# real-stanford/dgdm

Measured on AMD Instinct MI355X. Metric: guided samples/sec (full DDIM chain), higher is better.
Workload: dtype f32_split_f16x3; 1 GPU; 3d_guided BASELINE configs[2] (configs[3] at 8 GPUs): B=32 G=45 P=5 R=36000 sub_bs=512 N=512 T=15/S=5, fresh object per pair; contraction_flag=f32, fingers_per_pair=32, denoise_steps=5, rows_per_cond_fn=36000, cond_fn_per_chain_step=1, eps_net_form=f32_f16x3 batched, parallelism=pairs-sharded x1

## Files before the change

dgdm_amd/csrc/guidance_api.hip:

```cpp
#include "common.h"
#include "models.h"
#include <algorithm>
#include <cmath>
#include <cstring>
#include <unordered_map>
#include <atomic>
#include <thread>

using namespace dgdm;

namespace {

std::vector<float> linspace_f32(float start, float end, int steps) {
    std::vector<float> v(steps);
    if (steps == 1) { v[0] = start; return v; }
    const float step = (end - start) / (float)(steps - 1);
    const int half = steps / 2;
    for (int i = 0; i < steps; ++i) v[i] = i < half ? start + step * (float)i : end - step * (float)(steps - i - 1);
    return v;
}

struct ObjectTables {
    const float *xyz = nullptr;
    const int   *fps1 = nullptr;
// ... 40 lines not shown
    DevBuf pool_fps1t;
    DevBuf tmpY[NBUILD], tmpL2[NBUILD], vlist;
    DevBuf tmpShare[NBUILD];
    hipStream_t bstream[NBUILD] = {};
    hipEvent_t bev[NBUILD] = {}, bstart = nullptr, pooled = nullptr, ldone = nullptr;
    DevBuf V, genc, atab, chainbias, timepart, ttmp, ttmp64, partial, objdev, objidx, xobj, xobj16, starts, order, xchains, todo, groupoff;
    DevBuf loopx[2], loopeps, loopgrad, loopxrep, loopts;
    DevBuf loopeps1;
    DevBuf loopkeys;
    std::vector<uint64_t> loopkeys_host;
    DevBuf loopcond, loopx2, loopeps2;
    DevBuf scorelogits;
    DevBuf valobj;
    DevBuf sweep_ori, rollstate, rolllogits, rolltiles, rollpmax;
    const float *rowfield = nullptr;
    int rowfield_chains = 0;
    DevBuf pos_lin, goalspecs;
    DevBuf labelx, labelcounts, labelsums, labelfinal, labelfirst, labelleft, labelobj;
    int rolltiles_chains = 0;
    DevBuf xidx, xidxchains, xtabptrs;
    DevBuf l1ptrs, l1objs;
    bool l1tab = true;
    int fill_l1ptrs(const std::vector<const ObjectTables *> &of_chain, int *n_tabled, hipStream_t s);
    bool xtab_enabled = true;
    int xtab_policy = 0;
    int grads_since_set = 0;
    static constexpr int XTAB_AFTER = 5;
    int l2_gather_mode = 0;
    int xobj_mode = 0;
    int n_objects = 0;
    bool force_slow_xobj = false;
    void *pinned = nullptr; size_t pinned_bytes = 0; hipEvent_t pinned_ev = nullptr;
    int64_t todo_capacity = 0;
    int *ro_host = nullptr; size_t ro_ints = 0; hipEvent_t ro_ev = nullptr; bool ro_pending = false;
    int finish_objects();
    hipStream_t cstream = nullptr; hipEvent_t up_ready = nullptr, up_consumed = nullptr; bool consumed_recorded = false;
    int serial = 0;
    bool tables_off_stream() const { return !(serial & 3) && !prof_on(); }
    bool eps_beside() const { return !(serial & 5) && !prof_on(); }
    bool hoist_x_only() const { return !(serial & 1) && !prof_on(); }
    bool built_off_stream = false, join_pending = false, built_once = false;
    hipStream_t joined_stream = nullptr;
    hipEvent_t fork_ev = nullptr, side_ev = nullptr;
    int join_tables(hipStream_t s) {
        if (!built_off_stream || (!join_pending && s == joined_stream)) return DGDM_OK;
        DGDM_HIP_CHECK(hipStreamWaitEvent(s, ro_ev, 0));
        join_pending = false; joined_stream = s;
        return DGDM_OK;
    }
    int side_stream(hipStream_t *side) {
        if (!bstream[0]) DGDM_HIP_CHECK(hipStreamCreateWithFlags(&bstream[0], hipStreamNonBlocking));
        if (!fork_ev) DGDM_HIP_CHECK(hipEventCreateWithFlags(&fork_ev, hipEventDisableTiming));
        if (!side_ev) DGDM_HIP_CHECK(hipEventCreateWithFlags(&side_ev, hipEventDisableTiming));
        *side = bstream[0];
        return DGDM_OK;
    }
    ~DgdmGuidance() {
        for (int i = 0; i < NBUILD; ++i)
            if (bstream[i]) (void)hipStreamSynchronize(bstream[i]);
        if (fork_ev) (void)hipEventDestroy(fork_ev);
        if (side_ev) (void)hipEventDestroy(side_ev);
        if (pinned) (void)hipHostFree(pinned);
        if (pinned_ev) (void)hipEventDestroy(pinned_ev);
        if (ro_host) (void)hipHostFree(ro_host);
        if (ro_ev) (void)hipEventDestroy(ro_ev);
        if (cstream) (void)hipStreamDestroy(cstream);
        if (up_ready) (void)hipEventDestroy(up_ready);
        if (up_consumed) (void)hipEventDestroy(up_consumed);
        for (int i = 0; i < NBUILD; ++i) {
            if (bstream[i]) (void)hipStreamDestroy(bstream[i]);
            if (bev[i]) (void)hipEventDestroy(bev[i]);
        }
        if (bstart) (void)hipEventDestroy(bstart);
        if (ldone) (void)hipEventDestroy(ldone);
        if (pooled) (void)hipEventDestroy(pooled);
    }
    int build_pose_table(const std::vector<float> &ori, const std::vector<float> &pos, PoseGrid *dst, hipStream_t s);
    void set_grid(dgdm::TrunkParams *p, const PoseGrid &g, int n_chains) const;
    int check_objects(const int *oidx, int n_chains) const;
    bool tables_wanted() const { return xtab_enabled && !force_slow_xobj && xobj_mode == 0; }
    int common_pre(const float *x_dev, float t_scaled, const int *objidx_host, int n_chains, hipStream_t s);
    int upload_starts(const int64_t *starts_host, int n_chains, int64_t rows, hipStream_t s, bool need_order = true, int n_calls = 1,
                      int64_t call_stride = 0);
    int ensure_rows(int n_chains, int64_t rows_per_chain);
    int use_xtab(const int *objidx_host, int n_chains, int64_t rows, bool want16, int *l1, hipStream_t s);
    int build_object(int oi, int slot, hipStream_t s);
    int build_xtab(int oi, hipStream_t s);
    int run_xobj(const int *objidx_host, int n_chains, int64_t rows, bool want16, bool *used16, bool *via_tab, int *l1, hipStream_t s);
    struct Embedded {
        bool tab = false, used16 = false;
        int l1 = 0;
        int64_t rows_per_chain = 0;
        void point(dgdm::TrunkParams *p, const DgdmGuidance &g, int call, int64_t rows_per_call) const;
    };
    int embed_rows(const int *objidx_host, int n_chains, const int64_t *starts_host, int64_t rows_per_call, int n_calls, int64_t call_stride,
                   bool want16, Embedded *e, hipStream_t s);
    int embed(const int *objidx_host, int n_chains, const int64_t *starts_host, int n_calls, int64_t call_stride, Embedded *e, hipStream_t s);
    int trunk_front(int kind, const float *x_dev, int timestep, const int *objidx_host, const int64_t *starts_host, int n_chains, const Embedded *emb,
                    int call, dgdm::TrunkParams *p, hipStream_t s, bool pre_done = false);
};

int DgdmGuidance::build_pose_table(const std::vector<float> &ori, const std::vector<float> &pos, PoseGrid *dst, hipStream_t s) {
    const int n = (int)ori.size(), W1 = m->W1;
    dst->cells = n; dst->tiles_per_b = (n + 31) / 32; dst->rows = (int64_t)B * n;
    DevBuf d_ori, d_pos, d_emb;
    int rc;
    if ((rc = d_ori.upload(ori.data(), sizeof(float) * n))) return rc;
    if ((rc = d_pos.upload(pos.data(), sizeof(float) * 2 * n))) return rc;
    if ((rc = d_emb.alloc(sizeof(float) * 27 * n))) return rc;
    if ((rc = dst->tab.alloc(sizeof(float) * (size_t)W1 * n))) return rc;
    if ((rc = pose_embed(d_ori.as<float>(), d_pos.as<float>(), d_emb.as<float>(), n, s))) return rc;
    if ((rc = linear64(d_emb.as<float>(), nullptr, 27, m->blob64.at(m->off64.w1p_wt), nullptr, nullptr, 1, nullptr, dst->tab.as<float>(), W1, n, 27, W1, ACT_NONE, s))) return rc;
    if ((rc = dst->tiled.alloc(sizeof(float) * (size_t)W1 * dst->tiles_per_b * 32))) return rc;
    if ((rc = tile_table(dst->tab.as<float>(), n, W1, dst->tiled.as<float>(), s))) return rc;
    DGDM_HIP_CHECK(hipStreamSynchronize(s));
    return DGDM_OK;
// ... 232 lines not shown
            (rc = g->pool_pairs.alloc(no * N * N * sizeof(int))) || (rc = g->pool_rank.alloc(no * N * N * sizeof(short))) ||
            (rc = g->pool_F1.alloc(no * N * 128 * 8)) || (rc = g->pool_U.alloc(no * N * 128 * 8)) ||
            (rc = g->pool_fps1t.alloc(no * N * 64 * sizeof(uint4))))
            return rc;
        const bool l1 = g->l1tab && !g->bf16 && N >= 128;
        const size_t l1mo = (size_t)std::max(1, g->cfg.max_objects);
        if (l1) {
            std::vector<const void *> ptrs(3 * l1mo, nullptr);
            for (int i = 0; i < (int)g->tables.size(); ++i) {
                ObjectTables &t = *g->tables[i];
                if ((rc = t.M0.alloc((size_t)N * 256 * 4)) || (rc = t.L1Z.alloc((size_t)N * 512 * 4)) || (rc = t.L1K.alloc((size_t)N * sizeof(int)))) return rc;
                ptrs[i] = t.M0.p; ptrs[l1mo + i] = t.L1Z.p; ptrs[2 * l1mo + i] = t.L1K.p;
            }
            if ((rc = g->l1objs.alloc(sizeof(void *) * ptrs.size()))) return rc;
            DGDM_HIP_CHECK(hipMemcpyAsync(g->l1objs.p, ptrs.data(), sizeof(void *) * ptrs.size(), hipMemcpyHostToDevice, s));
        }
        for (int i = 0; i < n_objects; ++i) g->tables[i]->has_l1 = l1;
        if (!g->pooled) DGDM_HIP_CHECK(hipEventCreateWithFlags(&g->pooled, hipEventDisableTiming));
        DGDM_HIP_CHECK(hipMemcpyAsync(g->pool_xyz.p, objects_dev, no * N * 3 * 4, hipMemcpyDeviceToDevice, s));
        DGDM_HIP_CHECK(hipEventRecord(g->pooled, s));
        hipStream_t fs = s;
        if (off) {
            fs = g->bstream[ns - 1];
            for (int i = 1; i < ns; ++i) {
                DGDM_HIP_CHECK(hipStreamWaitEvent(g->bstream[i], g->pooled, 0));
                if (g->built_once) DGDM_HIP_CHECK(hipStreamWaitEvent(g->bstream[i], g->ro_ev, 0));
            }
        }
        if ((rc = pn_fps_tables(g->pool_xyz.as<float>(), N, N, g->pool_fps1.as<int>(), g->pool_fps2.as<int>(), g->pool_flags.as<int>(), fs, n_objects)))
            return rc;
        if (!g->bf16 && !g->l2_gather_mode && N <= 512 &&
            (rc = pn_fps_transpose(g->pool_fps1.as<int>(), N, g->pool_fps1t.as<uint4>(), fs, n_objects))) return rc;
        DGDM_HIP_CHECK(hipEventRecord(g->bstart, fs));
        for (int i = 0; i < n_objects; ++i) {
            ObjectTables &t = *g->tables[i];
            t.xyz = g->pool_xyz.as<float>() + (size_t)i * N * 3; t.fps1 = g->pool_fps1.as<int>() + (size_t)i * N * 512;
            t.fps2 = g->pool_fps2.as<int>() + (size_t)i * N * 128; t.flags = g->pool_flags.as<int>() + (size_t)i * N;
            t.crowded = g->pool_crowded.as<int>() + (size_t)i * N; t.clist = g->pool_clist.as<int>() + (size_t)i * (N + 1);
        }
        {
            hipStream_t ls = g->bstream[0];
            DGDM_HIP_CHECK(hipStreamWaitEvent(ls, g->pooled, 0));
            const PnWeights w = g->m->pn();
            if ((rc = pn_crowd(g->pool_xyz.as<float>(), N, w, g->pool_crowded.as<int>(), g->pool_clist.as<int>(), g->pool_clist.as<int>() + N,
                               g->pool_off.as<int>(), g->pool_pairs.as<int>(), g->pool_rank.as<short>(), ls, g->pool_ncr.as<int>(), n_objects)))
                return rc;
            if (g->bf16) {
                if ((rc = pn_sa1(g->pool_xyz.as<float>(), N, w, g->pool_F1.as<float>(), ls, n_objects))) return rc;
                if ((rc = linear(g->pool_F1.as<float>(), 128, w.sa2_wf_t, w.sa2_b0, nullptr, 1, g->pool_U.as<float>(), 128, n_objects * N, 128, 128,
                                 ACT_NONE, false, ls))) return rc;
            } else {
                const PnWeights64 w64 = g->m->pn64();
                if ((rc = pn_sa1_64(g->pool_xyz.as<float>(), N, w.r1sq, w64, g->pool_F1.as<double>(), ls, n_objects))) return rc;
                if ((rc = linear64(nullptr, g->pool_F1.as<double>(), 128, w64.sa2_wf_t, w64.sa2_b0, nullptr, 1, g->pool_U.as<double>(), nullptr, 128,
                                   n_objects * N, 128, 128, ACT_NONE, ls))) return rc;
            }
            DGDM_HIP_CHECK(hipEventRecord(g->ldone, ls));
        }
        for (int i = 0; i < nb; ++i) {
            DGDM_HIP_CHECK(hipStreamWaitEvent(g->bstream[i], g->bstart, 0));
            DGDM_HIP_CHECK(hipStreamWaitEvent(g->bstream[i], g->ldone, 0));
        }
        for (int i = 0; i < n_objects; ++i)
            if ((rc = g->build_object(i, i % nb, g->bstream[i % nb]))) return rc;
        hipStream_t es = off ? g->bstream[0] : s;
        for (int i = off ? 1 : 0; i < nb; ++i) {
            DGDM_HIP_CHECK(hipEventRecord(g->bev[i], g->bstream[i]));
            DGDM_HIP_CHECK(hipStreamWaitEvent(es, g->bev[i], 0));
        }
        if (l1) {
            void *const *po = g->l1objs.as<void *>();
            if ((rc = trunk_f16l_l1_tables(reinterpret_cast<const float *const *>(po), g->pool_ncr.as<int>(), reinterpret_cast<float *const *>(po + l1mo),
                                           reinterpret_cast<int *const *>(po + 2 * l1mo), N, n_objects, g->m->fwdh(), es))) return rc;
        }
        prof_end(s, DGDM_STAGE_TABLES, 0.0);
        const size_t need = no * N + no;
        if (need > g->ro_ints) {
            if (g->ro_host) DGDM_HIP_CHECK(hipHostFree(g->ro_host));
            g->ro_host = nullptr;
            DGDM_HIP_CHECK(hipHostMalloc(reinterpret_cast<void **>(&g->ro_host), need * sizeof(int), hipHostMallocDefault));
            g->ro_ints = need;
        }
        if (!g->ro_ev) DGDM_HIP_CHECK(hipEventCreateWithFlags(&g->ro_ev, hipEventDisableTiming));
        DGDM_HIP_CHECK(hipMemcpyAsync(g->ro_host, g->pool_flags.p, sizeof(int) * no * N, hipMemcpyDeviceToHost, es));
        DGDM_HIP_CHECK(hipMemcpyAsync(g->ro_host + no * N, g->pool_ncr.p, sizeof(int) * no, hipMemcpyDeviceToHost, es));
        DGDM_HIP_CHECK(hipEventRecord(g->ro_ev, es));
        g->ro_pending = true;
        g->built_once = true; g->built_off_stream = off; g->join_pending = off;
    }
    g->n_objects = n_objects;
    g->grads_since_set = 0;
    return DGDM_OK;
}

int DgdmGuidance::common_pre(const float *x_dev, float t_scaled, const int *objidx_host, int n_chains, hipStream_t s) {
    const int rows = n_chains * B, W1 = m->W1;
    int rc;
    if ((rc = m->gripper_forward64(x_dev, m->L, V.as<double>(), genc.as<double>(), rows, s))) return rc;
    if ((rc = m->time_part64(t_scaled, ttmp.as<float>(), ttmp64.as<double>(), timepart.as<double>(), s))) return rc;
    if (m->kind == 2) {
        DGDM_HIP_CHECK(hipMemcpyAsync(objidx.p, objidx_host, sizeof(int) * n_chains, hipMemcpyHostToDevice, s));
        if ((rc = gather_add64(objpart.as<double>(), objidx.as<int>(), timepart.as<double>(), chainbias.as<double>(), n_chains, W1, s))) return rc;
        return linear64(nullptr, genc.as<double>(), 256, m->blob64.at(m->off64.w1c_wt), nullptr, chainbias.as<double>(), B, nullptr, atab.as<float>(), W1, rows, 256, W1,
                        ACT_NONE, s);
    }
    return linear64(nullptr, genc.as<double>(), 256, m->blob64.at(m->off64.w1c_wt), timepart.as<double>(), nullptr, 1, nullptr, atab.as<float>(), W1, rows, 256, W1,
                    ACT_NONE, s);
}

int DgdmGuidance::finish_objects() {
    if (!ro_pending) return DGDM_OK;
    DGDM_HIP_CHECK(hipEventSynchronize(ro_ev));
    const int N = cfg.num_object_points;
    for (int i = 0; i < n_objects; ++i) {
        bool ok = N >= 128;
        for (int k = 0; k < N; ++k) ok = ok && ro_host[(size_t)i * N + k] == 0;
        tables[i]->fast_ok = ok;
        tables[i]->ncr = ro_host[(size_t)n_objects * N + i];
    }
    ro_pending = false;
    return DGDM_OK;
}

int DgdmGuidance::ensure_rows(int n_chains, int64_t rows_per_chain) {
    const int N = cfg.num_object_points;
    const size_t nr = (size_t)n_chains * rows_per_chain;
    int rc;
    if ((rc = starts.alloc(nr * 2 * sizeof(int))) || (rc = order.alloc(nr * sizeof(int))) ||
        (rc = todo.alloc((nr + 1) * sizeof(int))) || (rc = xidx.alloc(nr * sizeof(int))))
        return rc;
    todo_capacity = (int64_t)nr;
    const size_t need = (nr * 3 + (size_t)n_chains * (N + 1)) * sizeof(int);
    if (need > pinned_bytes) {
        if (pinned) { DGDM_HIP_CHECK(hipEventSynchronize(pinned_ev)); DGDM_HIP_CHECK(hipHostFree(pinned)); pinned = nullptr; pinned_bytes = 0; }
        DGDM_HIP_CHECK(hipHostMalloc(&pinned, need, hipHostMallocDefault));
        pinned_bytes = need;
    }
    return DGDM_OK;
}

int DgdmGuidance::upload_starts(const int64_t *starts_host, int n_chains, int64_t rows, hipStream_t s, bool need_order, int n_calls,
                                int64_t call_stride) {
    const int N = cfg.num_object_points;
    const int64_t sb = cfg.sub_batch_size;
    const int64_t rt = rows * n_calls;
    int rc;
    DGDM_REQUIRE(!need_order || rt < ((int64_t)1 << 22), DGDM_EINVAL, "%lld rows per chain in one gather launch (limit 4194303)", (long long)rt);
    if ((rc = ensure_rows(n_chains, rt))) return rc;
    DGDM_HIP_CHECK(hipEventSynchronize(pinned_ev));
    int *dst = static_cast<int *>(pinned);
    int *ord = dst + (size_t)n_chains * 2 * rt;
    int *goff = ord + (size_t)n_chains * rt;
    std::atomic<int> bad{0};
    auto work = [&](int c0, int c1) {
        std::vector<int> cnt(N + 1), cnt2(513), tmp;
        for (int c = c0; c < c1; ++c) {
            int *d = dst + (size_t)c * 2 * rt;
            for (int k = 0; k < n_calls; ++k) {
                const int64_t *src = starts_host + (size_t)k * call_stride + (size_t)c * 2 * rows;
                int *dk = d + 2 * (size_t)k * rows;
                for (int64_t r0 = 0; r0 < rows; r0 += sb) {
                    const int64_t n = std::min(sb, rows - r0);
                    const int64_t *s1 = src + 2 * r0, *s2 = s1 + n;
                    for (int64_t i = 0; i < n; ++i) {
                        const int64_t a = s1[i], b = s2[i];
                        if (!(a >= 0 && a < N && b >= 0 && b < 512)) { bad.store(1); return; }
                        dk[2 * (r0 + i)] = (int)a; dk[2 * (r0 + i) + 1] = (int)b;
                    }
                }
            }
            if (!need_order) continue;
            int *o = ord + (size_t)c * rt;
            tmp.resize((size_t)rt);
            std::fill(cnt2.begin(), cnt2.end(), 0);
            for (int64_t r = 0; r < rt; ++r) ++cnt2[d[2 * r + 1] + 1];
            for (int k = 0; k < 512; ++k) cnt2[k + 1] += cnt2[k];
            for (int64_t r = 0; r < rt; ++r) tmp[cnt2[d[2 * r + 1]]++] = (int)r;
            std::fill(cnt.begin(), cnt.end(), 0);
            for (int64_t r = 0; r < rt; ++r) ++cnt[d[2 * r] + 1];
            for (int k = 0; k < N; ++k) cnt[k + 1] += cnt[k];
            memcpy(goff + (size_t)c * (N + 1), cnt.data(), sizeof(int) * (N + 1));
            for (int64_t i = 0; i < rt; ++i) { const int r = tmp[i]; o[cnt[d[2 * r]]++] = r | (d[2 * r + 1] << 22); }
        }
    };
    const int hw = (int)std::max(2u, std::thread::hardware_concurrency());
    const int nthreads = (int)std::min<int64_t>(std::min(16, hw / 2), std::max<int64_t>(1, std::min<int64_t>(n_chains, (int64_t)n_chains * rt / 65536)));
    if (nthreads <= 1) {
        work(0, n_chains);
    } else {
        std::vector<std::thread> pool;
        for (int t = 0; t < nthreads; ++t) pool.emplace_back(work, (int)((int64_t)n_chains * t / nthreads), (int)((int64_t)n_chains * (t + 1) / nthreads));
        for (auto &th : pool) th.join();
    }
    DGDM_REQUIRE(!bad.load(), DGDM_EINVAL, "FPS start out of range (sa1 must be in [0, %d), sa2 in [0, 512))", N);
    if (!cstream) {
        DGDM_HIP_CHECK(hipStreamCreateWithFlags(&cstream, hipStreamNonBlocking));
        DGDM_HIP_CHECK(hipEventCreateWithFlags(&up_ready, hipEventDisableTiming));
        DGDM_HIP_CHECK(hipEventCreateWithFlags(&up_consumed, hipEventDisableTiming));
    }
    if (consumed_recorded) DGDM_HIP_CHECK(hipStreamWaitEvent(cstream, up_consumed, 0));
    DGDM_HIP_CHECK(hipMemcpyAsync(starts.p, pinned, (size_t)n_chains * rt * 2 * sizeof(int), hipMemcpyHostToDevice, cstream));
    if (need_order) {
        DGDM_HIP_CHECK(hipMemcpyAsync(order.p, ord, (size_t)n_chains * rt * sizeof(int), hipMemcpyHostToDevice, cstream));
        DGDM_HIP_CHECK(hipMemcpyAsync(groupoff.p, goff, (size_t)n_chains * (N + 1) * sizeof(int), hipMemcpyHostToDevice, cstream));
    }
    DGDM_HIP_CHECK(hipEventRecord(pinned_ev, cstream));
    DGDM_HIP_CHECK(hipEventRecord(up_ready, cstream));
    DGDM_HIP_CHECK(hipStreamWaitEvent(s, up_ready, 0));
    return DGDM_OK;
}

int DgdmGuidance::fill_l1ptrs(const std::vector<const ObjectTables *> &of_chain, int *n_tabled, hipStream_t s) {
    const int nc = cfg.max_chains;
    std::vector<const void *> ptrs(3 * (size_t)nc, nullptr);
    int *list = reinterpret_cast<int *>(ptrs.data() + 2 * (size_t)nc);
    std::vector<int> rest;
    int nt = 0;
    for (size_t i = 0; i < of_chain.size(); ++i) {
        const ObjectTables *t = of_chain[i];
        if (!t || !l1tab || !t->has_l1 || t->ncr != 0) { rest.push_back((int)i); continue; }
        ptrs[i] = t->L1Z.p; ptrs[nc + i] = t->L1K.p;
        list[nt++] = (int)i;
    }
    std::copy(rest.begin(), rest.end(), list + nt);
    *n_tabled = nt;
    if (nt) DGDM_HIP_CHECK(hipMemcpyAsync(l1ptrs.p, ptrs.data(), sizeof(void *) * ptrs.size(), hipMemcpyHostToDevice, s));
    return DGDM_OK;
}

int DgdmGuidance::use_xtab(const int *objidx_host, int n_chains, int64_t rows, bool want16, int *l1, hipStream_t s) {
    std::vector<XidxChain> xc(n_chains);
    std::vector<const void *> base(n_chains);
    std::vector<const ObjectTables *> m0_of(n_chains, nullptr);
    for (int i = 0; i < n_chains; ++i) {
        const ObjectTables &t = *tables[objidx_host[i]];
        xc[i].fps1 = t.fps1; xc[i].N = cfg.num_object_points; xc[i].m0_only = t.ncr == 0;
        base[i] = want16 ? (t.ncr == 0 ? (const void *)t.M0_16.p : (const void *)t.X16.p) : (t.ncr == 0 ? (const void *)t.M0.p : (const void *)t.X.p);
        if (!want16 && t.ncr == 0) m0_of[i] = &t;
    }
    int rc;
    if ((rc = fill_l1ptrs(m0_of, l1, s))) return rc;
// ... 3 lines not shown
}

int DgdmGuidance::run_xobj(const int *objidx_host, int n_chains, int64_t rows, bool want16, bool *used16, bool *via_tab, int *l1, hipStream_t s) {
    *via_tab = false;
    *l1 = 0;
    std::vector<XobjChain> ch(n_chains);
    for (int i = 0; i < n_chains; ++i) {
        const ObjectTables &t = *tables[objidx_host[i]];
        ch[i].xyz = t.xyz; ch[i].fps1 = t.fps1; ch[i].slot_of_start = nullptr; ch[i].Z = t.Z.as<float>();
        ch[i].fps2 = t.fps2; ch[i].flags = t.flags; ch[i].crowded = t.crowded; ch[i].N = cfg.num_object_points;
        ch[i].M0 = t.M0.as<float>(); ch[i].cl2 = t.cl2.as<int>(); ch[i].cnt2 = t.cnt2.as<int>();
        ch[i].Z16 = t.has16 ? t.Z16.as<uint32_t>() : nullptr; ch[i].M0_16 = t.has16 ? t.M0_16.as<uint32_t>() : nullptr;
        want16 = want16 && t.has16;
    }
    {
        const size_t nrows = (size_t)n_chains * rows;
        int rc = want16 ? xobj16.alloc(nrows * 512) : xobj.alloc(nrows * 256 * 4);
        if (rc) return rc;
    }
    *used16 = want16;
    XobjParams xp{};
    xp.chains = xchains.as<XobjChain>(); xp.starts = starts.as<int>(); xp.order = order.as<int>(); xp.xobj = xobj.as<float>();
    xp.xobj16 = want16 ? xobj16.as<uint32_t>() : nullptr;
    xp.R = rows; xp.total_rows = rows * n_chains; xp.use_table = force_slow_xobj ? 0 : 1;
    xp.todo = todo.as<int>(); xp.todo_count = todo.as<int>() + todo_capacity; xp.todo_capacity = todo_capacity;
    bool all_fast = true;
    for (int i = 0; i < n_chains; ++i) all_fast = all_fast && tables[objidx_host[i]]->fast_ok;
    bool groups = !force_slow_xobj && xobj_mode == 0 && cfg.num_object_points >= 128;
    for (int i = 0; i < n_chains && groups; ++i) {
        const ObjectTables &t = *tables[objidx_host[i]];
        const int lpr = xobj_rows_lpr(t.ncr, want16);
        groups = lpr > 0 && want16 == t.has16;
        ch[i].clist = t.clist; ch[i].cl2s = t.cl2s.as<int>(); ch[i].cl2o = t.cl2o.as<unsigned short>(); ch[i].pcf = t.pcf.as<int>(); ch[i].ncr = t.ncr; ch[i].lpr = lpr;
    }
    DGDM_HIP_CHECK(hipMemcpyAsync(xchains.p, ch.data(), sizeof(XobjChain) * n_chains, hipMemcpyHostToDevice, s));
    if (groups) {
        const bool by_index = tables_wanted() && (want16 || !bf16);
        std::vector<int> rank;
        std::vector<XidxChain> xc(n_chains);
        std::vector<const void *> base(n_chains);
        std::vector<const ObjectTables *> m0_of(n_chains, nullptr);
        for (int i = 0; i < n_chains; ++i) {
            const ObjectTables &t = *tables[objidx_host[i]];
            const bool m0_only = by_index && t.ncr == 0 && t.fast_ok;
            if (!m0_only) rank.push_back(i);
            if (m0_only && !want16) m0_of[i] = &t;
            xc[i].fps1 = m0_only ? t.fps1 : nullptr; xc[i].N = cfg.num_object_points; xc[i].m0_only = 1;
            base[i] = m0_only ? (want16 ? (const void *)t.M0_16.p : (const void *)t.M0.p)
                              : (want16 ? (const void *)(xobj16.as<uint32_t>() + (size_t)i * rows * 128) : (const void *)(xobj.as<float>() + (size_t)i * rows * 256));
        }
        xp.group_off = groupoff.as<int>(); xp.nchain = n_chains; xp.group_N = cfg.num_object_points; xp.use_table = 1;
        xp.total_items = (int)rank.size() * xp.group_N;
        std::stable_sort(rank.begin(), rank.end(), [&](int a, int b) { return ch[a].ncr > ch[b].ncr; });
        for (size_t i = 0; i < rank.size(); ++i) xp.chain_of_rank[i] = (unsigned char)rank[i];
        int rc = pn_xobj_groups(xp, s);
        if (rc || !by_index) return rc;
        *via_tab = true;
        DGDM_HIP_CHECK(hipMemcpyAsync(xidxchains.p, xc.data(), sizeof(XidxChain) * n_chains, hipMemcpyHostToDevice, s));
        DGDM_HIP_CHECK(hipMemcpyAsync(xtabptrs.p, base.data(), sizeof(void *) * n_chains, hipMemcpyHostToDevice, s));
        if ((rc = fill_l1ptrs(m0_of, l1, s))) return rc;
        return pn_xidx(xidxchains.as<XidxChain>(), starts.as<int>(), rows, n_chains, xidx.as<int>(), s);
    }
    return pn_xobj(xp, all_fast, s);
}

int DgdmGuidance::embed_rows(const int *oidx, int n_chains, const int64_t *starts_host, int64_t rows_per_call, int n_calls, int64_t call_stride,
                             bool want16, Embedded *e, hipStream_t s) {
    bool tab = tables_wanted();
    for (int i = 0; i < n_chains && tab; ++i) tab = want16 ? tables[oidx[i]]->has_x16 : tables[oidx[i]]->has_x;
    const int64_t rt = rows_per_call * n_calls;
    int rc;
    if ((rc = join_tables(s))) return rc;
    if ((rc = upload_starts(starts_host, n_chains, rows_per_call, s, !tab, n_calls, call_stride))) return rc;
    if ((rc = finish_objects())) return rc;
    e->tab = tab; e->used16 = want16; e->rows_per_chain = rt;
    if ((rc = tab ? use_xtab(oidx, n_chains, rt, want16, &e->l1, s) : run_xobj(oidx, n_chains, rt, want16, &e->used16, &e->tab, &e->l1, s))) return rc;
    DGDM_HIP_CHECK(hipEventRecord(up_consumed, s));
    consumed_recorded = true;
    return DGDM_OK;
}

void DgdmGuidance::Embedded::point(TrunkParams *p, const DgdmGuidance &g, int call, int64_t rows_per_call) const {
    const size_t row0 = (size_t)call * rows_per_call;
    p->xstride = rows_per_chain;
    if (tab) {
        p->xidx = g.xidx.as<int>() + row0;
        if (used16) p->xtab16 = g.xtabptrs.as<const uint32_t *>();
        else p->xtab = g.xtabptrs.as<const float *>();
        if (l1 && !used16) {
            p->l1z = g.l1ptrs.as<const float *>();
            p->l1k = g.l1ptrs.as<const int *>() + g.cfg.max_chains;
            p->chainlist = reinterpret_cast<const int *>(g.l1ptrs.as<const void *>() + 2 * (size_t)g.cfg.max_chains);
            p->n_tabled = l1;
        }
    } else {
        p->xobj = g.xobj.as<float>() + row0 * 256;
        p->xobj16 = used16 ? g.xobj16.as<uint32_t>() + row0 * 128 : nullptr;
    }
}

int DgdmGuidance::embed(const int *oidx, int n_chains, const int64_t *starts_host, int n_calls, int64_t call_stride, Embedded *e, hipStream_t s) {
    DGDM_REQUIRE(starts_host, DGDM_EINVAL, "3-D guidance needs the FPS start indices");
    int rc;
    if ((rc = join_tables(s))) return rc;
    prof_begin(s, DGDM_STAGE_XOBJ);
    if (tables_wanted()) {
        const bool crosses = grads_since_set <= XTAB_AFTER && grads_since_set + n_calls > XTAB_AFTER;
        grads_since_set += n_calls;
        if (crosses)
            for (int i = 0; i < n_objects; ++i) {
                ObjectTables &t = *tables[i];
                if (!(t.has16 ? t.has_x16 : t.has_x) && (rc = build_xtab(i, s))) return rc;
            }
    }
    if ((rc = embed_rows(oidx, n_chains, starts_host, grid.rows, n_calls, call_stride, bf16, e, s))) return rc;
    prof_end(s, DGDM_STAGE_XOBJ, 0.0);
    return DGDM_OK;
}

int DgdmGuidance::trunk_front(int kind, const float *x_dev, int timestep, const int *oidx, const int64_t *starts_host, int n_chains, const Embedded *emb,
                              int call, TrunkParams *pp, hipStream_t s, bool pre_done) {
    const float t_scaled = (float)timestep / (float)cfg.num_train_timesteps;
    int rc;
    if ((rc = check_objects(oidx, n_chains))) return rc;
    if (!pre_done) {
        prof_begin(s, DGDM_STAGE_GUIDE_MISC);
        if ((rc = common_pre(x_dev, t_scaled, oidx, n_chains, s))) return rc;
        prof_end(s, DGDM_STAGE_GUIDE_MISC, 0.0);
    }
    m->fill_trunk(pp);
    set_grid(pp, grid, n_chains);
    if (kind == 3) {
        Embedded own;
        if (!emb) {
            if ((rc = embed(oidx, n_chains, starts_host, 1, 0, &own, s))) return rc;
            emb = &own;
            call = 0;
        }
        emb->point(pp, *this, call, grid.rows);
    }
    return DGDM_OK;
// ... 617 lines not shown
```

dgdm_amd/csrc/pointnet.h:

```cpp
#pragma once
#include "common.h"

namespace dgdm {

struct PnWeights {
    float r1sq, r2sq;
    const float *sa1_w0t;
    const float *sa1_b0;
    const float *sa1_w1;
    const float *sa1_b1;
    const float *sa2_wf_t;
    const float *sa2_b0;
    const float *sa2_vx;
    const float4 *sa2_w1_img;
    const float *sa2_b1;
    const float4 *sa3_w_img16;
    const float *sa3_wx;
    const float *sa3_b;
};

struct PnWeights64 {
    const double *sa1_w0t, *sa1_b0, *sa1_w1, *sa1_b1;
    const double *sa2_wf_t, *sa2_b0, *sa2_vx;
    const double *sa2_w1_img, *sa2_b1;
// ... 60 lines not shown
    const uint4 *fps1t;
    unsigned char *sel;
    unsigned char *cnt;
    short *rep;
    int   *items;
    int   *coff, *ccnt;
    int   *nitems;
};
int pn_fps_table(const float *xyz, int N, int nv, int npoint, int *out, int *flags, hipStream_t s, int nobj = 1);
int pn_fps_tables(const float *xyz, int N, int nv, int *fps1, int *fps2, int *flags, hipStream_t s, int nobj = 1);
int pn_fps_transpose(const int *fps1, int nv, uint4 *fps1t, hipStream_t s, int nobj = 1);
int pn_sa1(const float *xyz, int N, const PnWeights &w, float *F1, hipStream_t s, int nobj = 1);
int pn_crowd(const float *xyz, int N, const PnWeights &w, int *crowded, int *clist, int *ncr, int *off, int *pairs, short *rank, hipStream_t s,
             int *ncr_copy = nullptr, int nobj = 1);
int pn_pairs(const float *xyz, int N, const float *U, const PnWeights &w, const int *pairs, const int *off, float *Y, uint32_t *Y16, hipStream_t s);
int pn_l2(const float *xyz, int N, const PnWeights &w, const int *fps1, const int *vlist, int nv, const float *Y, float *L2,
          const int *clist, const int *ncr, const int *off, const short *rank, bool bf16 , hipStream_t s,
          int crowded_mode = 0, const L2Share *share = nullptr);
int pn_z16(const float *xyz, int N, int nv, const PnWeights &w, const uint32_t *L2_16, float *Z, uint32_t *Z16, const int *clist, const int *ncr,
           hipStream_t s);
int pn_sa1_64(const float *xyz, int N, float r1sq, const PnWeights64 &w, double *F1_64, hipStream_t s, int nobj = 1);
int pn_pairs64(const float *xyz, int N, const double *U64, const PnWeights64 &w, const int *pairs, const int *off, float *Y, hipStream_t s);
int pn_z64(const float *xyz, int N, int nv, const PnWeights64 &w, const float *L2, float *Z, const int *clist, const int *ncr, hipStream_t s,
           const int *items = nullptr, const int *nitems = nullptr);
int pn_zfill(int N, int nv, float *Z, const int *clist, const int *ncr, const short *rep, hipStream_t s);
int pn_m0(const int *fps2, const int *crowded, int N, const float *Z0, float *M0, int *cl2, int *cnt2, const uint32_t *Z0_16, uint32_t *M0_16,
          const int *clist, const int *ncr, int *cl2s, unsigned short *cl2o, hipStream_t s);
__host__ __device__ inline int xobj_rows_lpr(int ncr, bool bf16) {
    for (int lpr = bf16 ? 32 : 64; lpr >= 8; lpr >>= 1)
        if (ncr * lpr * 16 <= 65536) return lpr;
    return 0;
}
int pn_xobj_groups(const XobjParams &p, hipStream_t s);
int pn_pcf(const int *fps1, const int *cnt2, const int *flags, int N, int *pcf, hipStream_t s);
int pn_debug_indices(const float *xyz, int N, const PnWeights &w, const int *perm, int M, int *ball1, int *ball2, int *ball2_cnt, int *crowded,
                     hipStream_t s);
int pn_xobj(const XobjParams &p, bool all_fast, hipStream_t s);

}
```

dgdm_amd/csrc/pointnet.hip:

```cpp
#include "common.h"
#include "mfma_chain.h"
#include <type_traits>
#include "pointnet.h"
#include "pointnet_dev.h"

#pragma clang fp contract(off)

namespace dgdm {

template <class T, class Op>
__device__ __forceinline__ T dpp_reduce(T v, Op op) {
    auto step = [&](auto ctrl, auto rmask) {
        constexpr int C = decltype(ctrl)::value, M = decltype(rmask)::value;
        const int o = __builtin_amdgcn_update_dpp(__builtin_bit_cast(int, v), __builtin_bit_cast(int, v), C, M, 0xf, false);
        v = op(v, __builtin_bit_cast(T, o));
    };
    step(std::integral_constant<int, 0xB1>{}, std::integral_constant<int, 0xf>{});
    step(std::integral_constant<int, 0x4E>{}, std::integral_constant<int, 0xf>{});
    step(std::integral_constant<int, 0x141>{}, std::integral_constant<int, 0xf>{});
    step(std::integral_constant<int, 0x140>{}, std::integral_constant<int, 0xf>{});
    step(std::integral_constant<int, 0x142>{}, std::integral_constant<int, 0xa>{});
    step(std::integral_constant<int, 0x143>{}, std::integral_constant<int, 0xc>{});
    return __builtin_bit_cast(T, __builtin_amdgcn_readlane(__builtin_bit_cast(int, v), 63));
}
// ... 1023 lines not shown
                int k2 = kk;
                do {
                    const int r = rid[k2];
                    if (!slow) *reinterpret_cast<__attribute__((address_space(1))) u4 *>(out + (size_t)r * W + f0) = best;
                    else if (chunk == 0 && fl == 0) p.todo[atomicAdd(p.todo_count, 1)] = (int)((int64_t)chain * p.R + r);
                    ++k2;
                } while (k2 < np && !(cfs[k2] & 512));
                li = li2; have = have2; kk = kk2; q = q2; cf = cf2; m0 = m02; cur = cur2; nx1 = nx12;
            }
        }
    }
}

template <bool BF16>
__global__ __launch_bounds__(64 * XR_WAVES, 4) void xobj_rows_kernel(const XobjParams p) {
    extern __shared__ unsigned char xr_lds[];
    const int N = p.group_N;
    const int chain = p.chain_of_rank[blockIdx.x / N], s1 = blockIdx.x % N;
    const XobjChain ch = p.chains[chain];
    switch (ch.lpr) {
        case 64: if (!BF16) xobj_rows_body<BF16, (BF16 ? 32 : 64)>(p, ch, chain, s1, xr_lds); break;
        case 32: xobj_rows_body<BF16, 32>(p, ch, chain, s1, xr_lds); break;
        case 16: xobj_rows_body<BF16, 16>(p, ch, chain, s1, xr_lds); break;
        default: xobj_rows_body<BF16, 8>(p, ch, chain, s1, xr_lds); break;
    }
}

int pn_pcf(const int *fps1, const int *cnt2, const int *flags, int N, int *pcf, hipStream_t s) {
    hipLaunchKernelGGL(pcf_kernel, dim3((unsigned)((N * 512 + 255) / 256)), dim3(256), 0, s, fps1, cnt2, flags, N, pcf);
    DGDM_HIP_CHECK(hipGetLastError());
    return DGDM_OK;
}

int pn_xobj_groups(const XobjParams &p, hipStream_t s) {
    if (p.total_items <= 0) return DGDM_OK;
    static bool attr_set = false;
    if (!attr_set) {
        DGDM_HIP_CHECK(hipFuncSetAttribute((const void *)xobj_rows_kernel<false>, hipFuncAttributeMaxDynamicSharedMemorySize, XR_LDS_BYTES));
        DGDM_HIP_CHECK(hipFuncSetAttribute((const void *)xobj_rows_kernel<true>, hipFuncAttributeMaxDynamicSharedMemorySize, XR_LDS_BYTES));
        attr_set = true;
    }
    DGDM_HIP_CHECK(hipMemsetAsync(p.todo_count, 0, sizeof(int), s));
    if (p.xobj16) hipLaunchKernelGGL(xobj_rows_kernel<true>, dim3((unsigned)p.total_items), dim3(64 * XR_WAVES), XR_LDS_BYTES, s, p);
    else hipLaunchKernelGGL(xobj_rows_kernel<false>, dim3((unsigned)p.total_items), dim3(64 * XR_WAVES), XR_LDS_BYTES, s, p);
    DGDM_HIP_CHECK(hipGetLastError());
    XobjParams q = p;
    q.skip_fast = 1;
    const int64_t cap = std::min<int64_t>(std::min<int64_t>(p.total_rows, p.todo_capacity), 8192);
    if (p.xobj16) hipLaunchKernelGGL(xobj_kernel<true>, dim3((unsigned)((cap + 3) / 4)), dim3(256), 0, s, q);
    else hipLaunchKernelGGL(xobj_kernel<false>, dim3((unsigned)((cap + 3) / 4)), dim3(256), 0, s, q);
    DGDM_HIP_CHECK(hipGetLastError());
    return DGDM_OK;
}

constexpr int XG_LDS_BYTES = 78 * 1024;

template <bool BF16, int LPR>
__device__ __forceinline__ void xtab_body(const XtabObj &o, int ncr, int s1, int chunk, uint32_t *slab) {
    typedef uint32_t u4 __attribute__((ext_vector_type(4)));
    constexpr int W = BF16 ? 128 : 256, F = 4 * LPR, RPW = 64 / LPR;
    const int lane = threadIdx.x & 63, wave = __builtin_amdgcn_readfirstlane(threadIdx.x >> 6);
    const int f0 = chunk * F, N = o.N;
    const uint32_t *Zs = (BF16 ? o.Z16 : reinterpret_cast<const uint32_t *>(o.Z)) + ((size_t)s1 * N) * W + f0;
    const int pieces = ncr * LPR;
    for (int i0 = threadIdx.x; i0 < pieces; i0 += 256 * 8) {
        u4 v[8];
#pragma unroll
        for (int k = 0; k < 8; ++k) {
            const int i = i0 + 256 * k;
            if (i < pieces) v[k] = *reinterpret_cast<const u4 *>(Zs + (size_t)o.clist[i / LPR] * W + (i % LPR) * 4);
        }
#pragma unroll
        for (int k = 0; k < 8; ++k) {
            const int i = i0 + 256 * k;
            if (i < pieces) *reinterpret_cast<u4 *>(slab + (size_t)i * 4) = v[k];
        }
    }
    __syncthreads();
// ... 439 lines not shown
```

Measured before the change: 21150 samples/s.

## Start per-object row gathers as each object's tables finish building

Splits the grouped xobj gather into begin/rows/ties phases and launches the row gather for each object once that object's build event fires, instead of waiting for the full table join. It also moves the host readback of flags and crowded counts earlier, right after the crowd stage on the side stream, and can upload starts on the launch stream. The goal is to overlap per-object table construction with embedding gathers and to shorten the critical path at the start of each fresh-object chain. It adds per-object events and more launches, and the synchronisation ordering gets more complex.

```diff
diff --git a/dgdm_amd/csrc/guidance_api.hip b/dgdm_amd/csrc/guidance_api.hip
--- a/dgdm_amd/csrc/guidance_api.hip
+++ b/dgdm_amd/csrc/guidance_api.hip
@@ -96,13 +96,15 @@
     bool force_slow_xobj = false;
     void *pinned = nullptr; size_t pinned_bytes = 0; hipEvent_t pinned_ev = nullptr;
     int64_t todo_capacity = 0;
-    int *ro_host = nullptr; size_t ro_ints = 0; hipEvent_t ro_ev = nullptr; bool ro_pending = false;
+    int *ro_host = nullptr; size_t ro_ints = 0; hipEvent_t ro_ev = nullptr, rb_ev = nullptr, crowd_ev = nullptr; bool ro_pending = false;
+    std::vector<hipEvent_t> odone;
     int finish_objects();
     hipStream_t cstream = nullptr; hipEvent_t up_ready = nullptr, up_consumed = nullptr; bool consumed_recorded = false;
     int serial = 0;
     bool tables_off_stream() const { return !(serial & 3) && !prof_on(); }
     bool eps_beside() const { return !(serial & 5) && !prof_on(); }
     bool hoist_x_only() const { return !(serial & 1) && !prof_on(); }
+    bool gather_early(hipStream_t s) const { return !(serial & 9) && !prof_on() && built_off_stream && (join_pending || s != joined_stream); }
     bool built_off_stream = false, join_pending = false, built_once = false;
     hipStream_t joined_stream = nullptr;
     hipEvent_t fork_ev = nullptr, side_ev = nullptr;
@@ -128,6 +130,9 @@
         if (pinned_ev) (void)hipEventDestroy(pinned_ev);
         if (ro_host) (void)hipHostFree(ro_host);
         if (ro_ev) (void)hipEventDestroy(ro_ev);
+        if (rb_ev) (void)hipEventDestroy(rb_ev);
+        if (crowd_ev) (void)hipEventDestroy(crowd_ev);
+        for (hipEvent_t e : odone) (void)hipEventDestroy(e);
         if (cstream) (void)hipStreamDestroy(cstream);
         if (up_ready) (void)hipEventDestroy(up_ready);
         if (up_consumed) (void)hipEventDestroy(up_consumed);
@@ -145,7 +150,7 @@
     bool tables_wanted() const { return xtab_enabled && !force_slow_xobj && xobj_mode == 0; }
     int common_pre(const float *x_dev, float t_scaled, const int *objidx_host, int n_chains, hipStream_t s);
     int upload_starts(const int64_t *starts_host, int n_chains, int64_t rows, hipStream_t s, bool need_order = true, int n_calls = 1,
-                      int64_t call_stride = 0);
+                      int64_t call_stride = 0, bool on_launch_stream = false);
     int ensure_rows(int n_chains, int64_t rows_per_chain);
     int use_xtab(const int *objidx_host, int n_chains, int64_t rows, bool want16, int *l1, hipStream_t s);
     int build_object(int oi, int slot, hipStream_t s);
@@ -444,6 +449,20 @@
         if (!g->bf16 && !g->l2_gather_mode && N <= 512 &&
             (rc = pn_fps_transpose(g->pool_fps1.as<int>(), N, g->pool_fps1t.as<uint4>(), fs, n_objects))) return rc;
         DGDM_HIP_CHECK(hipEventRecord(g->bstart, fs));
+        while ((int)g->odone.size() < n_objects) {
+            hipEvent_t e = nullptr;
+            DGDM_HIP_CHECK(hipEventCreateWithFlags(&e, hipEventDisableTiming));
+            g->odone.push_back(e);
+        }
+        if (!g->rb_ev) DGDM_HIP_CHECK(hipEventCreateWithFlags(&g->rb_ev, hipEventDisableTiming));
+        if (!g->crowd_ev) DGDM_HIP_CHECK(hipEventCreateWithFlags(&g->crowd_ev, hipEventDisableTiming));
+        const size_t ro_need = no * N + no;
+        if (ro_need > g->ro_ints) {
+            if (g->ro_host) { DGDM_HIP_CHECK(hipEventSynchronize(g->rb_ev)); DGDM_HIP_CHECK(hipHostFree(g->ro_host)); }
+            g->ro_host = nullptr; g->ro_ints = 0;
+            DGDM_HIP_CHECK(hipHostMalloc(reinterpret_cast<void **>(&g->ro_host), ro_need * sizeof(int), hipHostMallocDefault));
+            g->ro_ints = ro_need;
+        }
         for (int i = 0; i < n_objects; ++i) {
             ObjectTables &t = *g->tables[i];
             t.xyz = g->pool_xyz.as<float>() + (size_t)i * N * 3; t.fps1 = g->pool_fps1.as<int>() + (size_t)i * N * 512;
@@ -457,6 +476,7 @@
             if ((rc = pn_crowd(g->pool_xyz.as<float>(), N, w, g->pool_crowded.as<int>(), g->pool_clist.as<int>(), g->pool_clist.as<int>() + N,
                                g->pool_off.as<int>(), g->pool_pairs.as<int>(), g->pool_rank.as<short>(), ls, g->pool_ncr.as<int>(), n_objects)))
                 return rc;
+            DGDM_HIP_CHECK(hipEventRecord(g->crowd_ev, ls));
             if (g->bf16) {
                 if ((rc = pn_sa1(g->pool_xyz.as<float>(), N, w, g->pool_F1.as<float>(), ls, n_objects))) return rc;
                 if ((rc = linear(g->pool_F1.as<float>(), 128, w.sa2_wf_t, w.sa2_b0, nullptr, 1, g->pool_U.as<float>(), 128, n_objects * N, 128, 128,
@@ -469,12 +489,24 @@
             }
             DGDM_HIP_CHECK(hipEventRecord(g->ldone, ls));
         }
+        auto read_back = [&](hipStream_t rs) -> int {
+            DGDM_HIP_CHECK(hipMemcpyAsync(g->ro_host, g->pool_flags.p, sizeof(int) * no * N, hipMemcpyDeviceToHost, rs));
+            DGDM_HIP_CHECK(hipMemcpyAsync(g->ro_host + no * N, g->pool_ncr.p, sizeof(int) * no, hipMemcpyDeviceToHost, rs));
+            DGDM_HIP_CHECK(hipEventRecord(g->rb_ev, rs));
+            return DGDM_OK;
+        };
+        if (off) {
+            DGDM_HIP_CHECK(hipStreamWaitEvent(fs, g->crowd_ev, 0));
+            if ((rc = read_back(fs))) return rc;
+        }
         for (int i = 0; i < nb; ++i) {
             DGDM_HIP_CHECK(hipStreamWaitEvent(g->bstream[i], g->bstart, 0));
             DGDM_HIP_CHECK(hipStreamWaitEvent(g->bstream[i], g->ldone, 0));
         }
-        for (int i = 0; i < n_objects; ++i)
+        for (int i = 0; i < n_objects; ++i) {
             if ((rc = g->build_object(i, i % nb, g->bstream[i % nb]))) return rc;
+            DGDM_HIP_CHECK(hipEventRecord(g->odone[i], g->bstream[i % nb]));
+        }
         hipStream_t es = off ? g->bstream[0] : s;
         for (int i = off ? 1 : 0; i < nb; ++i) {
             DGDM_HIP_CHECK(hipEventRecord(g->bev[i], g->bstream[i]));
@@ -486,16 +518,9 @@
                                            reinterpret_cast<int *const *>(po + 2 * l1mo), N, n_objects, g->m->fwdh(), es))) return rc;
         }
         prof_end(s, DGDM_STAGE_TABLES, 0.0);
-        const size_t need = no * N + no;
-        if (need > g->ro_ints) {
-            if (g->ro_host) DGDM_HIP_CHECK(hipHostFree(g->ro_host));
-            g->ro_host = nullptr;
-            DGDM_HIP_CHECK(hipHostMalloc(reinterpret_cast<void **>(&g->ro_host), need * sizeof(int), hipHostMallocDefault));
-            g->ro_ints = need;
-        }
+        if (!off && (rc = read_back(es))) return rc;
+        if (off) DGDM_HIP_CHECK(hipStreamWaitEvent(es, g->rb_ev, 0));
         if (!g->ro_ev) DGDM_HIP_CHECK(hipEventCreateWithFlags(&g->ro_ev, hipEventDisableTiming));
-        DGDM_HIP_CHECK(hipMemcpyAsync(g->ro_host, g->pool_flags.p, sizeof(int) * no * N, hipMemcpyDeviceToHost, es));
-        DGDM_HIP_CHECK(hipMemcpyAsync(g->ro_host + no * N, g->pool_ncr.p, sizeof(int) * no, hipMemcpyDeviceToHost, es));
         DGDM_HIP_CHECK(hipEventRecord(g->ro_ev, es));
         g->ro_pending = true;
         g->built_once = true; g->built_off_stream = off; g->join_pending = off;
@@ -522,7 +547,7 @@
 
 int DgdmGuidance::finish_objects() {
     if (!ro_pending) return DGDM_OK;
-    DGDM_HIP_CHECK(hipEventSynchronize(ro_ev));
+    DGDM_HIP_CHECK(hipEventSynchronize(rb_ev));
     const int N = cfg.num_object_points;
     for (int i = 0; i < n_objects; ++i) {
         bool ok = N >= 128;
@@ -552,7 +577,7 @@
 }
 
 int DgdmGuidance::upload_starts(const int64_t *starts_host, int n_chains, int64_t rows, hipStream_t s, bool need_order, int n_calls,
-                                int64_t call_stride) {
+                                int64_t call_stride, bool on_launch_stream) {
     const int N = cfg.num_object_points;
     const int64_t sb = cfg.sub_batch_size;
     const int64_t rt = rows * n_calls;
@@ -610,15 +635,18 @@
         DGDM_HIP_CHECK(hipEventCreateWithFlags(&up_ready, hipEventDisableTiming));
         DGDM_HIP_CHECK(hipEventCreateWithFlags(&up_consumed, hipEventDisableTiming));
     }
-    if (consumed_recorded) DGDM_HIP_CHECK(hipStreamWaitEvent(cstream, up_consumed, 0));
-    DGDM_HIP_CHECK(hipMemcpyAsync(starts.p, pinned, (size_t)n_chains * rt * 2 * sizeof(int), hipMemcpyHostToDevice, cstream));
+    hipStream_t us = on_launch_stream ? s : cstream;
+    if (consumed_recorded) DGDM_HIP_CHECK(hipStreamWaitEvent(us, up_consumed, 0));
     if (need_order) {
-        DGDM_HIP_CHECK(hipMemcpyAsync(order.p, ord, (size_t)n_chains * rt * sizeof(int), hipMemcpyHostToDevice, cstream));
-        DGDM_HIP_CHECK(hipMemcpyAsync(groupoff.p, goff, (size_t)n_chains * (N + 1) * sizeof(int), hipMemcpyHostToDevice, cstream));
-    }
-    DGDM_HIP_CHECK(hipEventRecord(pinned_ev, cstream));
-    DGDM_HIP_CHECK(hipEventRecord(up_ready, cstream));
-    DGDM_HIP_CHECK(hipStreamWaitEvent(s, up_ready, 0));
+        DGDM_HIP_CHECK(hipMemcpyAsync(order.p, ord, (size_t)n_chains * rt * sizeof(int), hipMemcpyHostToDevice, us));
+        DGDM_HIP_CHECK(hipMemcpyAsync(groupoff.p, goff, (size_t)n_chains * (N + 1) * sizeof(int), hipMemcpyHostToDevice, us));
+    }
+    DGDM_HIP_CHECK(hipMemcpyAsync(starts.p, pinned, (size_t)n_chains * rt * 2 * sizeof(int), hipMemcpyHostToDevice, us));
+    DGDM_HIP_CHECK(hipEventRecord(pinned_ev, us));
+    if (!on_launch_stream) {
+        DGDM_HIP_CHECK(hipEventRecord(up_ready, cstream));
+        DGDM_HIP_CHECK(hipStreamWaitEvent(s, up_ready, 0));
+    }
     return DGDM_OK;
 }
 
@@ -688,6 +716,11 @@
         const int lpr = xobj_rows_lpr(t.ncr, want16);
         groups = lpr > 0 && want16 == t.has16;
         ch[i].clist = t.clist; ch[i].cl2s = t.cl2s.as<int>(); ch[i].cl2o = t.cl2o.as<unsigned short>(); ch[i].pcf = t.pcf.as<int>(); ch[i].ncr = t.ncr; ch[i].lpr = lpr;
+    }
+    const bool early = groups && gather_early(s);
+    if (!early) {
+        int rc = join_tables(s);
+        if (rc) return rc;
     }
     DGDM_HIP_CHECK(hipMemcpyAsync(xchains.p, ch.data(), sizeof(XobjChain) * n_chains, hipMemcpyHostToDevice, s));
     if (groups) {
@@ -706,16 +739,45 @@
                               : (want16 ? (const void *)(xobj16.as<uint32_t>() + (size_t)i * rows * 128) : (const void *)(xobj.as<float>() + (size_t)i * rows * 256));
         }
         xp.group_off = groupoff.as<int>(); xp.nchain = n_chains; xp.group_N = cfg.num_object_points; xp.use_table = 1;
-        xp.total_items = (int)rank.size() * xp.group_N;
-        std::stable_sort(rank.begin(), rank.end(), [&](int a, int b) { return ch[a].ncr > ch[b].ncr; });
-        for (size_t i = 0; i < rank.size(); ++i) xp.chain_of_rank[i] = (unsigned char)rank[i];
-        int rc = pn_xobj_groups(xp, s);
-        if (rc || !by_index) return rc;
-        *via_tab = true;
-        DGDM_HIP_CHECK(hipMemcpyAsync(xidxchains.p, xc.data(), sizeof(XidxChain) * n_chains, hipMemcpyHostToDevice, s));
-        DGDM_HIP_CHECK(hipMemcpyAsync(xtabptrs.p, base.data(), sizeof(void *) * n_chains, hipMemcpyHostToDevice, s));
-        if ((rc = fill_l1ptrs(m0_of, l1, s))) return rc;
-        return pn_xidx(xidxchains.as<XidxChain>(), starts.as<int>(), rows, n_chains, xidx.as<int>(), s);
+        auto index = [&]() -> int {
+            int rc;
+            *via_tab = true;
+            DGDM_HIP_CHECK(hipMemcpyAsync(xidxchains.p, xc.data(), sizeof(XidxChain) * n_chains, hipMemcpyHostToDevice, s));
+            DGDM_HIP_CHECK(hipMemcpyAsync(xtabptrs.p, base.data(), sizeof(void *) * n_chains, hipMemcpyHostToDevice, s));
+            if ((rc = fill_l1ptrs(m0_of, l1, s))) return rc;
+            return pn_xidx(xidxchains.as<XidxChain>(), starts.as<int>(), rows, n_chains, xidx.as<int>(), s);
+        };
+        int rc;
+        if (!early) {
+            xp.total_items = (int)rank.size() * xp.group_N;
+            std::stable_sort(rank.begin(), rank.end(), [&](int a, int b) { return ch[a].ncr > ch[b].ncr; });
+            for (size_t i = 0; i < rank.size(); ++i) xp.chain_of_rank[i] = (unsigned char)rank[i];
+            if ((rc = pn_xobj_groups(xp, s)) || !by_index) return rc;
+            return index();
+        }
+        auto gathers = [&]() -> int {
+            int rc;
+            if (by_index) {
+                DGDM_HIP_CHECK(hipStreamWaitEvent(s, bstart, 0));
+                if ((rc = index())) return rc;
+            }
+            if (rank.empty()) return DGDM_OK;
+            if ((rc = pn_xobj_groups_begin(xp, s))) return rc;
+            for (int o = 0; o < n_objects; ++o) {
+                int n = 0;
+                for (int c : rank)
+                    if (objidx_host[c] == o) xp.chain_of_rank[n++] = (unsigned char)c;
+                if (!n) continue;
+                xp.total_items = n * xp.group_N;
+                DGDM_HIP_CHECK(hipStreamWaitEvent(s, odone[o], 0));
+                if ((rc = pn_xobj_groups_rows(xp, s))) return rc;
+            }
+            return DGDM_OK;
+        };
+        rc = gathers();
+        const int jrc = join_tables(s);
+        if (rc || jrc) return rc ? rc : jrc;
+        return rank.empty() ? DGDM_OK : pn_xobj_groups_ties(xp, s);
     }
     return pn_xobj(xp, all_fast, s);
 }
@@ -726,8 +788,8 @@
     for (int i = 0; i < n_chains && tab; ++i) tab = want16 ? tables[oidx[i]]->has_x16 : tables[oidx[i]]->has_x;
     const int64_t rt = rows_per_call * n_calls;
     int rc;
-    if ((rc = join_tables(s))) return rc;
-    if ((rc = upload_starts(starts_host, n_chains, rows_per_call, s, !tab, n_calls, call_stride))) return rc;
+    if (tab && (rc = join_tables(s))) return rc;
+    if ((rc = upload_starts(starts_host, n_chains, rows_per_call, s, !tab, n_calls, call_stride, !tab && gather_early(s)))) return rc;
     if ((rc = finish_objects())) return rc;
     e->tab = tab; e->used16 = want16; e->rows_per_chain = rt;
     if ((rc = tab ? use_xtab(oidx, n_chains, rt, want16, &e->l1, s) : run_xobj(oidx, n_chains, rt, want16, &e->used16, &e->tab, &e->l1, s))) return rc;
@@ -758,11 +820,12 @@
 int DgdmGuidance::embed(const int *oidx, int n_chains, const int64_t *starts_host, int n_calls, int64_t call_stride, Embedded *e, hipStream_t s) {
     DGDM_REQUIRE(starts_host, DGDM_EINVAL, "3-D guidance needs the FPS start indices");
     int rc;
-    if ((rc = join_tables(s))) return rc;
+    if (prof_on() && (rc = join_tables(s))) return rc;
     prof_begin(s, DGDM_STAGE_XOBJ);
     if (tables_wanted()) {
         const bool crosses = grads_since_set <= XTAB_AFTER && grads_since_set + n_calls > XTAB_AFTER;
         grads_since_set += n_calls;
+        if (crosses && (rc = join_tables(s))) return rc;
         if (crosses)
             for (int i = 0; i < n_objects; ++i) {
                 ObjectTables &t = *tables[i];
diff --git a/dgdm_amd/csrc/pointnet.h b/dgdm_amd/csrc/pointnet.h
--- a/dgdm_amd/csrc/pointnet.h
+++ b/dgdm_amd/csrc/pointnet.h
@@ -116,6 +116,9 @@
     return 0;
 }
 int pn_xobj_groups(const XobjParams &p, hipStream_t s);
+int pn_xobj_groups_begin(const XobjParams &p, hipStream_t s);
+int pn_xobj_groups_rows(const XobjParams &p, hipStream_t s);
+int pn_xobj_groups_ties(const XobjParams &p, hipStream_t s);
 int pn_pcf(const int *fps1, const int *cnt2, const int *flags, int N, int *pcf, hipStream_t s);
 int pn_debug_indices(const float *xyz, int N, const PnWeights &w, const int *perm, int M, int *ball1, int *ball2, int *ball2_cnt, int *crowded,
                      hipStream_t s);
diff --git a/dgdm_amd/csrc/pointnet.hip b/dgdm_amd/csrc/pointnet.hip
--- a/dgdm_amd/csrc/pointnet.hip
+++ b/dgdm_amd/csrc/pointnet.hip
@@ -1079,8 +1079,7 @@
     return DGDM_OK;
 }
 
-int pn_xobj_groups(const XobjParams &p, hipStream_t s) {
-    if (p.total_items <= 0) return DGDM_OK;
+int pn_xobj_groups_begin(const XobjParams &p, hipStream_t s) {
     static bool attr_set = false;
     if (!attr_set) {
         DGDM_HIP_CHECK(hipFuncSetAttribute((const void *)xobj_rows_kernel<false>, hipFuncAttributeMaxDynamicSharedMemorySize, XR_LDS_BYTES));
@@ -1088,9 +1087,25 @@
         attr_set = true;
     }
     DGDM_HIP_CHECK(hipMemsetAsync(p.todo_count, 0, sizeof(int), s));
+    return DGDM_OK;
+}
+
+int pn_xobj_groups_rows(const XobjParams &p, hipStream_t s) {
+    if (p.total_items <= 0) return DGDM_OK;
     if (p.xobj16) hipLaunchKernelGGL(xobj_rows_kernel<true>, dim3((unsigned)p.total_items), dim3(64 * XR_WAVES), XR_LDS_BYTES, s, p);
     else hipLaunchKernelGGL(xobj_rows_kernel<false>, dim3((unsigned)p.total_items), dim3(64 * XR_WAVES), XR_LDS_BYTES, s, p);
     DGDM_HIP_CHECK(hipGetLastError());
+    return DGDM_OK;
+}
+
+int pn_xobj_groups(const XobjParams &p, hipStream_t s) {
+    if (p.total_items <= 0) return DGDM_OK;
+    int rc;
+    if ((rc = pn_xobj_groups_begin(p, s)) || (rc = pn_xobj_groups_rows(p, s))) return rc;
+    return pn_xobj_groups_ties(p, s);
+}
+
+int pn_xobj_groups_ties(const XobjParams &p, hipStream_t s) {
     XobjParams q = p;
     q.skip_fast = 1;
     const int64_t cap = std::min<int64_t>(std::min<int64_t>(p.total_rows, p.todo_capacity), 8192);
```

Measured after the change: 21410 samples/s, median of 6. 1.2% higher.
